# toandaominh1997/EfficientDet.Pytorch

Measured on NVIDIA H100. Metric: EfficientDet-D0 512x512 images/sec (fwd+bwd), higher is better.
Workload: dtype f32

## Files before the change

efficientdet.pytorch_b200/csrc/conv_planes.cu:

```cuda
#include "tc_ptx.cuh"

#include <stdlib.h>

namespace effdet {

constexpr int kPlMaxLevels = 8;
constexpr int kPlThreads = 288;
constexpr int kPlA = 128 * 128;
template <int BN>
struct PlCfg {
    static constexpr int kStages = BN == 128 ? 3 : 4;
    static constexpr int kB = BN * 128;
    static constexpr int kStage = 2 * kPlA + 2 * kB;
    static constexpr int kSmem = kStages * kStage + kRowsBytes + 1024 + 256 + BN * 4;
};

struct PlLevel {
    int B, H, W;
    WgGeom g;
    int tile_begin;
    int nboxes;
    float* y;
    long long y_bstride;
    __nv_bfloat16* y_planes;
    const __nv_bfloat16* mask_planes;
    const float* residual;
    long long r_bstride;
};
struct PlArgs {
    PlLevel lv[kPlMaxLevels];
    int nlevels, total_tiles, ntn;
    int Cin, Cout, ksize, act, kblocks, opitch;
    const float* bias;
    float* colsum;
};
struct PlMaps {
    CUtensorMap x[kPlMaxLevels];
};

template <int BN>
__global__ void __launch_bounds__(kPlThreads, 1)
conv_planes_kernel(const __grid_constant__ PlMaps maps, const __grid_constant__ CUtensorMap wmap, const __grid_constant__ PlArgs P) {
    constexpr int kPlBN = BN, kPlStages = PlCfg<BN>::kStages, kPlB = PlCfg<BN>::kB, kPlStage = PlCfg<BN>::kStage;
    extern __shared__ uint8_t smem_raw[];
    uint8_t* smem = smem_raw + ((1024u - (smem_u32(smem_raw) & 1023u)) & 1023u);
    float* rows_buf = reinterpret_cast<float*>(smem + kPlStages * kPlStage);
    uint64_t* full_bar = reinterpret_cast<uint64_t*>(smem + kPlStages * kPlStage + kRowsBytes);
    uint64_t* empty_bar = full_bar + kPlStages;
    float* chan = reinterpret_cast<float*>(smem + kPlStages * kPlStage + kRowsBytes + 256);

    const int warp = threadIdx.x >> 5, lane = threadIdx.x & 31;
    const int taps = P.ksize * P.ksize, pad = P.ksize / 2;
    const int KT = taps * P.kblocks;
    if (threadIdx.x == 0) {
        for (int s = 0; s < kPlStages; ++s) {
            mbar_init(&full_bar[s], 1);
            mbar_init(&empty_bar[s], 8);
        }
        fence_barrier_init();
        tma_prefetch_desc(&wmap);
    }
    __syncthreads();

    auto decode = [&](int unit, int& l, int& box0, int& n0) {
        const int mt = unit / P.ntn;
        n0 = (unit - mt * P.ntn) * kPlBN;
        l = 0;
        while (l + 1 < P.nlevels && mt >= P.lv[l + 1].tile_begin) ++l;
        box0 = (mt - P.lv[l].tile_begin) * (128 / P.lv[l].g.kstage);
    };

    if (warp == 8) {
        if (lane == 0) {
            uint32_t it = 0;
            for (int unit = blockIdx.x; unit < P.total_tiles; unit += gridDim.x) {
                int l, box0, n0;
                decode(unit, l, box0, n0);
                const PlLevel& L = P.lv[l];
                const int ks = L.g.kstage, nbox = 128 / ks;
                const int nvalid = min(nbox, L.nboxes - box0);
                for (int kt = 0; kt < KT; ++kt, ++it) {
                    const int s = it % kPlStages;
                    const uint32_t ph = (it / kPlStages) & 1;
                    const int tap = kt / P.kblocks, kb = kt - tap * P.kblocks;
                    const int dy = tap / P.ksize - pad, dx = tap % P.ksize - pad;
                    mbar_wait(&empty_bar[s], ph ^ 1);
                    uint8_t* a_hi = smem + s * kPlStage;
                    uint8_t* b_hi = a_hi + 2 * kPlA;
                    mbar_arrive_expect_tx(&full_bar[s], (uint32_t)(2 * nvalid * ks * 128 + 2 * kPlB));
                    for (int q = 0; q < nvalid; ++q) {
                        int ch = box0 + q;
                        const int bx = ch % L.g.nbx;
                        ch /= L.g.nbx;
                        const int by = ch % L.g.nby;
                        const int bb = ch / L.g.nby;
                        const int x0 = bx * L.g.Wb + dx, y0 = by * L.g.Hb + dy, b0 = bb * L.g.Bb;
                        tma_load_5d(a_hi + q * ks * 128, &maps.x[l], &full_bar[s], kb * 64, x0, y0, b0, 0);
                        tma_load_5d(a_hi + kPlA + q * ks * 128, &maps.x[l], &full_bar[s], kb * 64, x0, y0, b0, 1);
                    }
                    tma_load_3d(b_hi, &wmap, &full_bar[s], kt * 64, n0, 0);
                    tma_load_3d(b_hi + kPlB, &wmap, &full_bar[s], kt * 64, n0, 1);
                }
            }
        }
    } else {
        constexpr int NB = kPlBN / 64;
        const int g = warp >> 2;
        const int etid = threadIdx.x;
        const int quarter = 2 * g + (warp & 1), half = (warp >> 1) & 1;
        const int r = quarter * 32 + lane;
        uint32_t it = 0;
        int chan_n0 = -1;
        for (int unit = blockIdx.x; unit < P.total_tiles; unit += gridDim.x) {
            int l, box0, n0;
            decode(unit, l, box0, n0);
            const PlLevel& L = P.lv[l];
            float d[NB][32];
            for (int kt = 0; kt < KT; ++kt, ++it) {
                const int s = it % kPlStages;
                const uint32_t ph = (it / kPlStages) & 1;
                mbar_wait(&full_bar[s], ph);
                const uint32_t sa = smem_u32(smem + s * kPlStage) + g * 64 * 128;
                const uint32_t sb = smem_u32(smem + s * kPlStage) + 2 * kPlA;
                wgmma_fence();
#pragma unroll
                for (int k = 0; k < 4; ++k)
                    wg_mma3<NB, 0>(d, sa + k * 32, sa + kPlA + k * 32, sb + k * 32, sb + kPlB + k * 32, 16, 1024, (kt | k) != 0);
                wgmma_commit();
                wgmma_wait<1>();
                if (kt > 0 && lane == 0) mbar_arrive(&empty_bar[(it - 1) % kPlStages]);
            }
            wgmma_wait<0>();
            if (lane == 0) mbar_arrive(&empty_bar[(it - 1) % kPlStages]);
            if (n0 != chan_n0) {
                named_bar_sync(1, 256);
                for (int i = etid; i < kPlBN; i += 256) chan[i] = (n0 + i < P.Cout && P.bias) ? __ldg(P.bias + n0 + i) : 0.f;
                named_bar_sync(1, 256);
                chan_n0 = n0;
            }
            const int ks = L.g.kstage;
            const int q = r / ks, i = r - q * ks;
            int ch = box0 + q;
            bool row_ok = ch < L.nboxes;
            const int bx = ch % L.g.nbx;
            ch /= L.g.nbx;
            const int by = ch % L.g.nby;
            const int bb = ch / L.g.nby;
            const int wh = L.g.Wb * L.g.Hb;
            const int bi = i / wh, rem = i - bi * wh;
            const int yy = rem / L.g.Wb, xx = rem - yy * L.g.Wb;
            const int b = bb * L.g.Bb + bi, y = by * L.g.Hb + yy, x = bx * L.g.Wb + xx;
            row_ok = row_ok && b < L.B;
            const long long pixb = (long long)y * L.W + x;
            const long long pix = (long long)b * L.H * L.W + pixb;
            const long long plane = (long long)L.B * L.H * L.W * P.opitch;
            const int ncols = min(kPlBN, P.Cout - n0);
            const int nchunks = (ncols + 31) >> 5;
#pragma unroll
            for (int jb = 0; jb < NB; ++jb) {
                float v[32];
                wg_rows<2>(d[jb], rows_buf, g, v);
                const int cc = 2 * jb + half;
                if (cc >= nchunks) continue;
                const int nb = n0 + cc * 32;
#pragma unroll
                for (int k = 0; k < 32; ++k) {
                    float t = v[k] + chan[cc * 32 + k];
                    if (P.act == EFFDET_ACT_RELU) t = fmaxf(t, 0.f);
                    else if (P.act == EFFDET_ACT_SIGMOID) t = sigmoidf_(t);
                    v[k] = t;
                }
                if (row_ok && L.residual) {
#pragma unroll
                    for (int k4 = 0; k4 < 8; ++k4) {
                        if (nb + k4 * 4 >= P.Cout) break;
                        const float4 rv = ldg4(L.residual + (long long)b * L.r_bstride + pixb * P.Cout + nb + k4 * 4);
                        v[k4 * 4] += rv.x; v[k4 * 4 + 1] += rv.y; v[k4 * 4 + 2] += rv.z; v[k4 * 4 + 3] += rv.w;
                    }
                }
                if (row_ok && L.mask_planes) {
                    const __nv_bfloat16* mh = L.mask_planes + pix * P.opitch + nb;
#pragma unroll
                    for (int k8 = 0; k8 < 4; ++k8) {
                        if (nb + k8 * 8 >= P.Cout) break;
                        const uint4 hv = __ldg(reinterpret_cast<const uint4*>(mh + k8 * 8));
                        const uint4 lv = __ldg(reinterpret_cast<const uint4*>(mh + plane + k8 * 8));
                        const uint32_t hw[4] = {hv.x, hv.y, hv.z, hv.w}, lw[4] = {lv.x, lv.y, lv.z, lv.w};
#pragma unroll
                        for (int e = 0; e < 8; ++e) {
                            const uint32_t hb = (hw[e >> 1] >> ((e & 1) * 16)) & 0xffffu, lb = (lw[e >> 1] >> ((e & 1) * 16)) & 0xffffu;
                            const bool pos = (hb & 0x7fffu) ? !(hb & 0x8000u) : ((lb & 0x7fffu) && !(lb & 0x8000u));
                            if (!pos) v[k8 * 8 + e] = 0.f;
                        }
                    }
                }
                if (!row_ok) {
#pragma unroll
                    for (int k = 0; k < 32; ++k) v[k] = 0.f;
                }
                if (row_ok && L.y) {
                    float* yo = L.y + (long long)b * L.y_bstride + pixb * P.Cout + nb;
#pragma unroll
                    for (int k4 = 0; k4 < 8; ++k4) {
                        if (nb + k4 * 4 >= P.Cout) break;
                        st4(yo + k4 * 4, make_float4(v[k4 * 4], v[k4 * 4 + 1], v[k4 * 4 + 2], v[k4 * 4 + 3]));
                    }
                }
                if (row_ok && L.y_planes) {
                    __nv_bfloat16* ph = L.y_planes + pix * P.opitch + nb;
#pragma unroll
                    for (int k8 = 0; k8 < 4; ++k8) {
                        if (nb + k8 * 8 >= P.Cout) break;
                        uint4 hi, lo;
                        split8(make_float4(v[k8 * 8], v[k8 * 8 + 1], v[k8 * 8 + 2], v[k8 * 8 + 3]),
                               make_float4(v[k8 * 8 + 4], v[k8 * 8 + 5], v[k8 * 8 + 6], v[k8 * 8 + 7]), hi, lo);
                        *reinterpret_cast<uint4*>(ph + k8 * 8) = hi;
                        *reinterpret_cast<uint4*>(ph + plane + k8 * 8) = lo;
                    }
                }
                if (P.colsum) {
#pragma unroll
                    for (int off = 16; off >= 1; off >>= 1) {
                        const bool upper = (lane & off) != 0;
#pragma unroll
                        for (int k = 0; k < off; ++k) {
                            const float send = upper ? v[k] : v[k + off];
                            const float keep = upper ? v[k + off] : v[k];
                            v[k] = keep + __shfl_xor_sync(0xffffffffu, send, off);
                        }
                    }
                    if (nb + lane < P.Cout) atomicAdd(P.colsum + nb + lane, v[0]);
                }
            }
        }
    }
}

__global__ void __launch_bounds__(256) to_planes_kernel(const float* __restrict__ x, long long x_bstride, const float* __restrict__ prob,
                                                        long long p_bstride, __nv_bfloat16* __restrict__ out, float* __restrict__ colsum,
                                                        int B, int HW, int C, int pitch, int rows_per_block) {
    __shared__ float red[256 * 8];
    const int cv8 = pitch / 8;
    const int cvb = cv8 < 256 ? cv8 : 256;
    const int rows = 256 / cvb;
    const int tr = threadIdx.x / cvb, tc = threadIdx.x - tr * cvb;
    const int j = blockIdx.y * cvb + tc;
    const bool active = tr < rows && j < cv8;
    const long long nrows = (long long)B * HW;
    const long long plane = nrows * pitch;
    float s[8];
#pragma unroll
    for (int i = 0; i < 8; ++i) s[i] = 0.f;
    if (active) {
        const int c = j * 8;
        const long long r_begin = (long long)blockIdx.x * rows_per_block;
        const long long r_end = min(nrows, r_begin + rows_per_block);
        for (long long row = r_begin + tr; row < r_end; row += rows) {
            const int b = (int)(row / HW);
            const long long pix = row - (long long)b * HW;
            float4 v0 = f4zero(), v1 = f4zero();
            if (c < C) {
                const float* q = x + (long long)b * x_bstride + pix * C + c;
                v0 = ldg4(q);
                if (c + 4 < C) v1 = ldg4(q + 4);
                if (prob) {
                    const float* pp = prob + (long long)b * p_bstride + pix * C + c;
                    const float4 p0 = ldg4(pp);
                    v0 = make_float4(v0.x * p0.x * (1.f - p0.x), v0.y * p0.y * (1.f - p0.y), v0.z * p0.z * (1.f - p0.z),
                                     v0.w * p0.w * (1.f - p0.w));
                    if (c + 4 < C) {
                        const float4 p1 = ldg4(pp + 4);
                        v1 = make_float4(v1.x * p1.x * (1.f - p1.x), v1.y * p1.y * (1.f - p1.y), v1.z * p1.z * (1.f - p1.z),
                                         v1.w * p1.w * (1.f - p1.w));
                    }
                }
            }
            uint4 hi, lo;
            split8(v0, v1, hi, lo);
            *reinterpret_cast<uint4*>(out + row * pitch + c) = hi;
            *reinterpret_cast<uint4*>(out + plane + row * pitch + c) = lo;
            s[0] += v0.x; s[1] += v0.y; s[2] += v0.z; s[3] += v0.w;
            s[4] += v1.x; s[5] += v1.y; s[6] += v1.z; s[7] += v1.w;
        }
    }
    if (colsum == nullptr) return;
#pragma unroll
    for (int i = 0; i < 8; ++i) red[threadIdx.x * 8 + i] = s[i];
    __syncthreads();
    if (tr == 0 && j < cv8) {
#pragma unroll
        for (int i = 0; i < 8; ++i) {
            float acc = 0.f;
            for (int rr = 0; rr < rows; ++rr) acc += red[(rr * cvb + tc) * 8 + i];
            const int c = j * 8 + i;
            if (c < C) atomicAdd(colsum + c, acc);
        }
    }
}

}

using namespace effdet;

extern "C" int effdet_to_planes(const float* x, int64_t x_bstride, const float* prob, int64_t p_bstride, void* planes,
                                float* colsum, int B, int HW, int C, int device, effdet_stream_t stream) {
    EFFDET_REQUIRE(x && planes && B > 0 && HW > 0 && C > 0 && C % 4 == 0, "to_planes: bad arguments");
    EFFDET_REQUIRE(aligned16(x) && aligned16(prob) && aligned16(planes) && x_bstride % 4 == 0 && p_bstride % 4 == 0,
                   "to_planes: alignment");
    EFFDET_DEVICE(device);
    const int pitch = (C + 7) / 8 * 8;
    const int cv8 = pitch / 8;
    const int cvb = cv8 < 256 ? cv8 : 256;
    const int rows = 256 / cvb;
    const long long nrows = (long long)B * HW;
    long long rpb = (nrows + num_sms() * 4 - 1) / (num_sms() * 4);
    if (rpb < (long long)rows * 8) rpb = (long long)rows * 8;
    dim3 grid(cdiv(nrows, rpb), cdiv(cv8, cvb));
    to_planes_kernel<<<grid, 256, 0, (cudaStream_t)stream>>>(x, x_bstride, prob, p_bstride, (__nv_bfloat16*)planes, colsum, B, HW, C,
                                                            pitch, (int)rpb);
    return launch_status("to_planes_kernel");
}

extern "C" int effdet_conv_planes_multi(const effdet_conv_planes_args* levels, int nlevels, int device, effdet_stream_t stream) {
    EFFDET_REQUIRE(levels && nlevels >= 1 && nlevels <= kPlMaxLevels, "conv_planes_multi: 1..%d levels", kPlMaxLevels);
    const effdet_conv_planes_args* a0 = &levels[0];
    EFFDET_REQUIRE(a0->w_tc && (a0->ksize == 1 || a0->ksize == 3) && a0->Cin % 4 == 0 && a0->Cout % 4 == 0 && a0->Cin >= 8 &&
                       a0->Cout >= 8,
                   "conv_planes_multi: needs the bf16 weight pack, k in {1,3}, channels %% 4 == 0");
    EncodeTiledFn enc = encode_fn();
    if (!enc) return fail(EFFDET_ERR_UNSUPPORTED, "conv_planes_multi: cuTensorMapEncodeTiled unavailable");
    EFFDET_DEVICE(device);
    PlMaps maps;
    PlArgs P;
    memset(&P, 0, sizeof(P));
    const int opitch = (a0->Cout + 7) / 8 * 8, ipitch = (a0->Cin + 7) / 8 * 8;
    int tiles = 0;
    for (int l = 0; l < nlevels; ++l) {
        const effdet_conv_planes_args* a = &levels[l];
        EFFDET_REQUIRE(a->x_planes && (a->y || a->y_planes), "conv_planes_multi: null tensor");
        EFFDET_REQUIRE(a->Cin == a0->Cin && a->Cout == a0->Cout && a->ksize == a0->ksize && a->act == a0->act && a->w_tc == a0->w_tc &&
                           a->bias == a0->bias && a->colsum == a0->colsum,
                       "conv_planes_multi: all levels must share weights, bias, channels and activation");
        EFFDET_REQUIRE(aligned16(a->x_planes) && aligned16(a->y) && aligned16(a->y_planes) && aligned16(a->mask_planes) &&
                           aligned16(a->residual) && a->y_bstride % 4 == 0 && a->r_bstride % 4 == 0,
                       "conv_planes_multi: alignment");
        PlLevel& L = P.lv[l];
        L.B = a->B; L.H = a->H; L.W = a->W;
        if (!wg_geometry(a->B, a->H, a->W, &L.g))
            return fail(EFFDET_ERR_UNSUPPORTED, "conv_planes_multi: a %dx%dx%d map has no legal pixel box (check effdet_wgrad_tc_geometry_ok)",
                        a->B, a->H, a->W);
        L.nboxes = L.g.nbx * L.g.nby * L.g.nbb;
        L.tile_begin = tiles;
        tiles += cdiv(L.nboxes, 128 / L.g.kstage);
        L.y = a->y; L.y_bstride = a->y_bstride;
        L.y_planes = (__nv_bfloat16*)a->y_planes;
        L.mask_planes = (const __nv_bfloat16*)a->mask_planes;
        L.residual = a->residual; L.r_bstride = a->r_bstride;
        int s = planes_map(enc, &maps.x[l], const_cast<void*>(a->x_planes), a->B, a->H, a->W, a->Cin, ipitch, L.g);
        if (s) return s;
    }
    for (int l = nlevels; l < kPlMaxLevels; ++l) {
        maps.x[l] = maps.x[0];
        P.lv[l].tile_begin = tiles;
    }
    const int taps = a0->ksize * a0->ksize;
    const int kpad = conv_tc_kpad(a0->Cin);
    const int BN = a0->Cout <= 64 ? 64 : 128;
    CUtensorMap wmap;
    {
        const cuuint64_t gdim[3] = {(cuuint64_t)taps * kpad, (cuuint64_t)a0->Cout, 2};
        const cuuint64_t gstr[2] = {(cuuint64_t)taps * kpad * 2, (cuuint64_t)a0->Cout * taps * kpad * 2};
        const cuuint32_t box[3] = {64, (cuuint32_t)BN, 1};
        const cuuint32_t estr[3] = {1, 1, 1};
        CUresult r = enc(&wmap, CU_TENSOR_MAP_DATA_TYPE_BFLOAT16, 3, const_cast<void*>(a0->w_tc), gdim, gstr, box, estr,
                         CU_TENSOR_MAP_INTERLEAVE_NONE, CU_TENSOR_MAP_SWIZZLE_128B, CU_TENSOR_MAP_L2_PROMOTION_L2_256B,
                         CU_TENSOR_MAP_FLOAT_OOB_FILL_NONE);
        if (r != CUDA_SUCCESS) return fail(EFFDET_ERR_LAUNCH, "conv_planes_multi: tensor map of the weights failed (%d)", (int)r);
    }
    P.nlevels = nlevels;
    P.ntn = cdiv(a0->Cout, BN);
    P.total_tiles = tiles * P.ntn;
    P.Cin = a0->Cin; P.Cout = a0->Cout; P.ksize = a0->ksize; P.act = a0->act;
    P.kblocks = kpad / 64;
    P.opitch = opitch;
    P.bias = a0->bias;
    P.colsum = a0->colsum;
    const int grid = P.total_tiles < num_sms() ? P.total_tiles : num_sms();
#define EFFDET_PL_LAUNCH(BN_)                                                                                              \
    do {                                                                                                                  \
        cudaError_t e = cudaFuncSetAttribute(conv_planes_kernel<BN_>, cudaFuncAttributeMaxDynamicSharedMemorySize,         \
                                             PlCfg<BN_>::kSmem);                                                          \
        if (e != cudaSuccess) return fail(EFFDET_ERR_LAUNCH, "conv_planes_multi: smem opt-in: %s", cudaGetErrorString(e)); \
        conv_planes_kernel<BN_><<<grid, kPlThreads, PlCfg<BN_>::kSmem, (cudaStream_t)stream>>>(maps, wmap, P);             \
    } while (0)
    if (BN == 64) EFFDET_PL_LAUNCH(64);
    else EFFDET_PL_LAUNCH(128);
#undef EFFDET_PL_LAUNCH
    return launch_status("conv_planes_kernel");
}
```

efficientdet.pytorch_b200/csrc/conv_tc.cu:

```cuda
#include "tc_ptx.cuh"

#include <stdlib.h>

namespace effdet {

constexpr int kTcThreads = 288;
constexpr int kTcProducers = 256;
constexpr int kFwdThreads = 288;
constexpr int kFwdProducers = 256;
constexpr int kTileM = 128;
constexpr int kTileK = 64;

template <int BN, int STAGES>
struct FwdSmem {
    static constexpr int kA = kTileM * 128;
    static constexpr int kB = BN * 128;
    static constexpr int kStage = 2 * kA + 2 * kB;
    static constexpr int kChan = 3 * BN * 4;
    static constexpr int kBytes = STAGES * kStage + 1024  + 256  + kChan;
};

template <int BN, int STAGES, bool MB>
__device__ __forceinline__ void conv_tc_body(const CUtensorMap& wmap, const effdet_conv_args& p, const int M, const int HW,
                                             const int kblocks, const int m0, const int n0) {
// ... 670 lines not shown
#define EFFDET_TC_LAUNCH(BN_, ST_)                                                                                         \
    do {                                                                                                                  \
        if (mb) EFFDET_TC_LAUNCH1(BN_, ST_, true);                                                                        \
        else EFFDET_TC_LAUNCH1(BN_, ST_, false);                                                                          \
    } while (0)
    if (KT <= 2) {
        if (BN == 64) EFFDET_TC_LAUNCH(64, 1);
        else EFFDET_TC_LAUNCH(128, 1);
    } else {
        if (BN == 64) EFFDET_TC_LAUNCH(64, 4);
        else EFFDET_TC_LAUNCH(128, 3);
    }
#undef EFFDET_TC_LAUNCH
#undef EFFDET_TC_LAUNCH1
    return launch_status("conv_tc_kernel");
}


int conv_tc_multi_launch(const effdet_conv_args* levels, int nlevels, cudaStream_t st) {
    EncodeTiledFn enc = encode_fn();
    if (!enc) return fail(EFFDET_ERR_UNSUPPORTED, "conv2d_multi(tc): cuTensorMapEncodeTiled unavailable");
    const effdet_conv_args* a = &levels[0];
    const int taps = a->ksize * a->ksize;
    const int kpad = conv_tc_kpad(a->Cin);
    const int kblocks = kpad / kTileK;
    const int BN = a->Cout <= 64 ? 64 : 128;
    CUtensorMap map;
    const cuuint64_t gdim[3] = {(cuuint64_t)taps * kpad, (cuuint64_t)a->Cout, 2};
    const cuuint64_t gstr[2] = {(cuuint64_t)taps * kpad * 2, (cuuint64_t)a->Cout * taps * kpad * 2};
    const cuuint32_t box[3] = {(cuuint32_t)kTileK, (cuuint32_t)BN, 1};
    const cuuint32_t estr[3] = {1, 1, 1};
    CUresult r = enc(&map, CU_TENSOR_MAP_DATA_TYPE_BFLOAT16, 3, const_cast<void*>(a->w_tc), gdim, gstr, box, estr,
                     CU_TENSOR_MAP_INTERLEAVE_NONE, CU_TENSOR_MAP_SWIZZLE_128B, CU_TENSOR_MAP_L2_PROMOTION_L2_256B,
                     CU_TENSOR_MAP_FLOAT_OOB_FILL_NONE);
    if (r != CUDA_SUCCESS) return fail(EFFDET_ERR_LAUNCH, "conv2d_multi(tc): cuTensorMapEncodeTiled failed (%d)", (int)r);
    ConvMultiArgs ma;
    memset(&ma, 0, sizeof(ma));
    ma.nlevels = nlevels;
    int tiles = 0;
    for (int l = 0; l < nlevels; ++l) {
        ma.lv[l] = levels[l];
        ma.tile_begin[l] = tiles;
        tiles += cdiv((long long)levels[l].B * levels[l].H * levels[l].W, kTileM);
    }
    for (int l = nlevels; l <= kMaxLevels; ++l) ma.tile_begin[l] = tiles;
    dim3 grid(tiles, cdiv(a->Cout, BN));
#define EFFDET_TCM_LAUNCH(BN_, ST_)                                                                                        \
    do {                                                                                                                  \
        cudaError_t e = cudaFuncSetAttribute(conv_tc_multi_kernel<BN_, ST_>, cudaFuncAttributeMaxDynamicSharedMemorySize,  \
                                             FwdSmem<BN_, ST_>::kBytes);                                                  \
        if (e != cudaSuccess) return fail(EFFDET_ERR_LAUNCH, "conv2d_multi(tc): smem opt-in: %s", cudaGetErrorString(e)); \
        conv_tc_multi_kernel<BN_, ST_><<<grid, kFwdThreads, FwdSmem<BN_, ST_>::kBytes, st>>>(map, ma, kblocks);            \
    } while (0)
    if (BN == 64) EFFDET_TCM_LAUNCH(64, 4);
    else EFFDET_TCM_LAUNCH(128, 3);
#undef EFFDET_TCM_LAUNCH
    return launch_status("conv_tc_multi_kernel");
}

bool wgrad_tc_eligible(const effdet_wgrad_args* a) {
    if (a->precision != 1 || a->Cin % 4 || a->Cout % 4 || a->Cin < 16 || a->Cout < 16) return false;
    WgGeom g;
    const bool tma_ok = (a->ws_x || a->x_planes) && (a->ws_dy || a->dy_planes) && wg_geometry(a->B, a->H, a->W, &g);
    return tma_ok || (!a->a_scale && !a->in_scale && !a->dy_planes && !a->x_planes);
}

bool wg_geometry(int B, int H, int W, WgGeom* g) {
    const int Wb = W <= 64 ? W : 64;
    if (W % Wb) return false;
    int Hb = 1;
    for (int h = 1; h <= H && Wb * h <= 64; ++h)
        if (H % h == 0) Hb = h;
    int Bb = 64 / (Wb * Hb);
    if (Bb < 1) Bb = 1;
    if (Bb > B) Bb = B;
    const int ks = Wb * Hb * Bb;
    if (ks < 16 || ks % 16) return false;
    g->Wb = Wb; g->Hb = Hb; g->Bb = Bb;
    g->nbx = W / Wb; g->nby = H / Hb; g->nbb = (B + Bb - 1) / Bb;
    g->kstage = ks;
    return true;
}

int planes_map(EncodeTiledFn enc, CUtensorMap* map, void* base, int B, int H, int W, int C, int pitch, const WgGeom& g) {
    const cuuint64_t gdim[5] = {(cuuint64_t)C, (cuuint64_t)W, (cuuint64_t)H, (cuuint64_t)B, 2};
    const cuuint64_t gstr[4] = {(cuuint64_t)pitch * 2, (cuuint64_t)W * pitch * 2, (cuuint64_t)H * W * pitch * 2,
                                (cuuint64_t)B * H * W * pitch * 2};
    const cuuint32_t box[5] = {64, (cuuint32_t)g.Wb, (cuuint32_t)g.Hb, (cuuint32_t)g.Bb, 1};
    const cuuint32_t estr[5] = {1, 1, 1, 1, 1};
    CUresult r = enc(map, CU_TENSOR_MAP_DATA_TYPE_BFLOAT16, 5, base, gdim, gstr, box, estr, CU_TENSOR_MAP_INTERLEAVE_NONE,
                     CU_TENSOR_MAP_SWIZZLE_128B, CU_TENSOR_MAP_L2_PROMOTION_L2_256B, CU_TENSOR_MAP_FLOAT_OOB_FILL_NONE);
    if (r != CUDA_SUCCESS) return fail(EFFDET_ERR_LAUNCH, "wgrad(tc): cuTensorMapEncodeTiled failed (%d)", (int)r);
    return EFFDET_OK;
}

static int wgrad_tc2_launch(const effdet_wgrad_args* a, cudaStream_t st) {
    WgGeom g;
    EncodeTiledFn enc = encode_fn();
    if (!enc || !(a->ws_x || a->x_planes) || !(a->ws_dy || a->dy_planes) || !wg_geometry(a->B, a->H, a->W, &g)) return 1;
    const int HW = a->H * a->W;
    const int cin_pad = conv_tc_kpad(a->Cin), cout_pad = conv_tc_kpad(a->Cout);
    int s = EFFDET_OK;
    if (!a->x_planes) {
        int blocks = cdiv((long long)a->B * HW * (cin_pad / 8), 256);
        if (blocks > num_sms() * 16) blocks = num_sms() * 16;
        split_planes_kernel<<<blocks, 256, 0, st>>>(a->x, a->x_bstride, a->a_scale, (__nv_bfloat16*)a->ws_x, a->B, HW, a->Cin, cin_pad,
                                                    a->in_scale, a->in_shift);
        s = launch_status("split_planes_kernel");
        if (s) return s;
    }
    CUtensorMap mdy, mx;
    if (a->dy_planes) {
        if ((s = planes_map(enc, &mdy, const_cast<void*>(a->dy_planes), a->B, a->H, a->W, a->Cout, (a->Cout + 7) / 8 * 8, g))) return s;
    } else {
        if ((s = split_dy_launch(a, cout_pad, st))) return s;
        if ((s = planes_map(enc, &mdy, a->ws_dy, a->B, a->H, a->W, cout_pad, cout_pad, g))) return s;
    }
    if (a->x_planes) {
        if ((s = planes_map(enc, &mx, const_cast<void*>(a->x_planes), a->B, a->H, a->W, a->Cin, (a->Cin + 7) / 8 * 8, g))) return s;
    } else {
        if ((s = planes_map(enc, &mx, a->ws_x, a->B, a->H, a->W, cin_pad, cin_pad, g))) return s;
    }
    const int taps = a->ksize * a->ksize;
    const int BC = a->Cin > 64 ? 256 : 64;
    const int ctiles = cdiv(a->Cin, BC), ntiles = cdiv(a->Cout, kTileM);
    const int nchunks = g.nbx * g.nby * g.nbb;
    int splits = (num_sms() * 2) / (ctiles * ntiles * taps);
    if (splits < 1) splits = 1;
    if (splits > cdiv(nchunks, 4)) splits = cdiv(nchunks, 4);
    int cps = cdiv(nchunks, splits);
    splits = cdiv(nchunks, cps);
    dim3 grid(ctiles * ntiles, taps, splits);
    cudaError_t e;
    if (BC == 256) {
        constexpr int ST = 2;
        e = cudaFuncSetAttribute(wgrad_tc2_kernel<256, ST>, cudaFuncAttributeMaxDynamicSharedMemorySize, WgSmem<256, ST>::kBytes);
        if (e != cudaSuccess) return fail(EFFDET_ERR_LAUNCH, "wgrad(tc): smem opt-in: %s", cudaGetErrorString(e));
        wgrad_tc2_kernel<256, ST><<<grid, kTcThreads, WgSmem<256, ST>::kBytes, st>>>(mdy, mx, *a, g, cps, ctiles);
    } else {
        constexpr int ST = 4;
        e = cudaFuncSetAttribute(wgrad_tc2_kernel<64, ST>, cudaFuncAttributeMaxDynamicSharedMemorySize, WgSmem<64, ST>::kBytes);
        if (e != cudaSuccess) return fail(EFFDET_ERR_LAUNCH, "wgrad(tc): smem opt-in: %s", cudaGetErrorString(e));
        wgrad_tc2_kernel<64, ST><<<grid, kTcThreads, WgSmem<64, ST>::kBytes, st>>>(mdy, mx, *a, g, cps, ctiles);
    }
    return launch_status("wgrad_tc2_kernel");
}

int wgrad_tc2_multi_launch(const effdet_wgrad_args* levels, int nlevels, cudaStream_t st) {
    EncodeTiledFn enc = encode_fn();
    if (!enc || nlevels > kWgMaxLevels) return 1;
    WgMaps maps;
    WgMultiArgs ma;
    memset(&ma, 0, sizeof(ma));
    const effdet_wgrad_args* a0 = &levels[0];
    const int cin_pad = conv_tc_kpad(a0->Cin), cout_pad = conv_tc_kpad(a0->Cout);
    int chunks = 0;
    for (int l = 0; l < nlevels; ++l) {
        const effdet_wgrad_args* a = &levels[l];
        if (!(a->ws_x || a->x_planes) || !(a->ws_dy || a->dy_planes) || a->a_scale || a->in_scale ||
            !wg_geometry(a->B, a->H, a->W, &ma.g[l]))
            return 1;
        ma.chunk_begin[l] = chunks;
        chunks += ma.g[l].nbx * ma.g[l].nby * ma.g[l].nbb;
    }
    for (int l = nlevels; l <= kWgMaxLevels; ++l) ma.chunk_begin[l] = chunks;
    ma.nlevels = nlevels;
    ma.dw = a0->dw;
    ma.Cin = a0->Cin; ma.Cout = a0->Cout; ma.ksize = a0->ksize;
    for (int l = 0; l < nlevels; ++l) {
        const effdet_wgrad_args* a = &levels[l];
        const int HW = a->H * a->W;
        int s = EFFDET_OK;
        if (a->x_planes) {
            if ((s = planes_map(enc, &maps.x[l], const_cast<void*>(a->x_planes), a->B, a->H, a->W, a->Cin, (a->Cin + 7) / 8 * 8, ma.g[l])))
// ... 168 lines not shown
```

efficientdet.pytorch_b200/csrc/tc_ptx.cuh:

```cuda
#pragma once
#include "common.cuh"

#include <cuda.h>
#include <cuda_bf16.h>
#include <type_traits>

namespace effdet {

__device__ __forceinline__ uint32_t smem_u32(const void* p) { return (uint32_t)__cvta_generic_to_shared(p); }

__device__ __forceinline__ void mbar_init(uint64_t* bar, uint32_t count) {
    asm volatile("mbarrier.init.shared::cta.b64 [%0], %1;" ::"r"(smem_u32(bar)), "r"(count));
}
__device__ __forceinline__ void mbar_arrive(uint64_t* bar) {
    asm volatile("mbarrier.arrive.shared::cta.b64 _, [%0];" ::"r"(smem_u32(bar)) : "memory");
}
__device__ __forceinline__ void mbar_arrive_expect_tx(uint64_t* bar, uint32_t bytes) {
    asm volatile("mbarrier.arrive.expect_tx.shared::cta.b64 _, [%0], %1;" ::"r"(smem_u32(bar)), "r"(bytes) : "memory");
}
__device__ __forceinline__ void mbar_wait(uint64_t* bar, uint32_t parity) {
    const uint32_t a = smem_u32(bar);
    uint32_t done;
    do {
        asm volatile(
            "{\n\t.reg .pred p;\n\t"
            "mbarrier.try_wait.parity.shared::cta.b64 p, [%1], %2;\n\t"
            "selp.u32 %0, 1, 0, p;\n\t}"
            : "=r"(done)
            : "r"(a), "r"(parity)
            : "memory");
    } while (!done);
}
__device__ __forceinline__ void fence_barrier_init() { asm volatile("fence.mbarrier_init.release.cluster;" ::: "memory"); }
__device__ __forceinline__ void fence_proxy_async() { asm volatile("fence.proxy.async.shared::cta;" ::: "memory"); }
__device__ __forceinline__ void tma_load_3d(void* dst, const CUtensorMap* map, uint64_t* bar, int c0, int c1, int c2) {
    asm volatile(
        "cp.async.bulk.tensor.3d.shared::cluster.global.tile.mbarrier::complete_tx::bytes [%0], [%1, {%3, %4, %5}], [%2];"
        ::"r"(smem_u32(dst)), "l"(reinterpret_cast<uint64_t>(map)), "r"(smem_u32(bar)), "r"(c0), "r"(c1), "r"(c2)
        : "memory");
}

__device__ __forceinline__ void tma_load_5d(void* dst, const CUtensorMap* map, uint64_t* bar, int c0, int c1, int c2, int c3, int c4) {
    asm volatile(
        "cp.async.bulk.tensor.5d.shared::cluster.global.tile.mbarrier::complete_tx::bytes [%0], [%1, {%3, %4, %5, %6, %7}], [%2];"
        ::"r"(smem_u32(dst)), "l"(reinterpret_cast<uint64_t>(map)), "r"(smem_u32(bar)), "r"(c0), "r"(c1), "r"(c2), "r"(c3), "r"(c4)
        : "memory");
}


__device__ __forceinline__ uint64_t gmma_desc(uint32_t smem_addr, uint32_t lbo_bytes, uint32_t sbo_bytes) {
    return (uint64_t)((smem_addr >> 4) & 0x3FFF) | ((uint64_t)((lbo_bytes >> 4) & 0x3FFF) << 16) |
           ((uint64_t)((sbo_bytes >> 4) & 0x3FFF) << 32) | (1ull << 62);
}
__device__ __forceinline__ void wgmma_fence() { asm volatile("wgmma.fence.sync.aligned;" ::: "memory"); }
__device__ __forceinline__ void wgmma_commit() { asm volatile("wgmma.commit_group.sync.aligned;" ::: "memory"); }
template <int N>
__device__ __forceinline__ void wgmma_wait() {
    asm volatile("wgmma.wait_group.sync.aligned %0;" ::"n"(N) : "memory");
}
#define EFFDET_WG_D8(a, o) "+f"(a[o]), "+f"(a[o + 1]), "+f"(a[o + 2]), "+f"(a[o + 3]), "+f"(a[o + 4]), "+f"(a[o + 5]), \
                           "+f"(a[o + 6]), "+f"(a[o + 7])
#define EFFDET_WG_D32(a) EFFDET_WG_D8(a, 0), EFFDET_WG_D8(a, 8), EFFDET_WG_D8(a, 16), EFFDET_WG_D8(a, 24)
template <int MN>
__device__ __forceinline__ void wgmma_bf16(float (&d)[1][32], uint64_t desc_a, uint64_t desc_b, uint32_t accumulate) {
    asm volatile(
        "{\n\t.reg .pred p;\n\t"
        "setp.ne.b32 p, %34, 0;\n\t"
        "wgmma.mma_async.sync.aligned.m64n64k16.f32.bf16.bf16 {"
        "%0, %1, %2, %3, %4, %5, %6, %7, %8, %9, %10, %11, %12, %13, %14, %15, "
        "%16, %17, %18, %19, %20, %21, %22, %23, %24, %25, %26, %27, %28, %29, %30, %31"
        "}, %32, %33, p, 1, 1, %35, %35;\n\t}"
        : EFFDET_WG_D32(d[0])
        : "l"(desc_a), "l"(desc_b), "r"(accumulate), "n"(MN)
        : "memory");
}
template <int MN>
__device__ __forceinline__ void wgmma_bf16(float (&d)[2][32], uint64_t desc_a, uint64_t desc_b, uint32_t accumulate) {
    asm volatile(
        "{\n\t.reg .pred p;\n\t"
        "setp.ne.b32 p, %66, 0;\n\t"
        "wgmma.mma_async.sync.aligned.m64n128k16.f32.bf16.bf16 {"
        "%0, %1, %2, %3, %4, %5, %6, %7, %8, %9, %10, %11, %12, %13, %14, %15, "
        "%16, %17, %18, %19, %20, %21, %22, %23, %24, %25, %26, %27, %28, %29, %30, %31, "
        "%32, %33, %34, %35, %36, %37, %38, %39, %40, %41, %42, %43, %44, %45, %46, %47, "
        "%48, %49, %50, %51, %52, %53, %54, %55, %56, %57, %58, %59, %60, %61, %62, %63"
        "}, %64, %65, p, 1, 1, %67, %67;\n\t}"
        : EFFDET_WG_D32(d[0]), EFFDET_WG_D32(d[1])
        : "l"(desc_a), "l"(desc_b), "r"(accumulate), "n"(MN)
        : "memory");
}
template <int MN>
__device__ __forceinline__ void wgmma_bf16(float (&d)[4][32], uint64_t desc_a, uint64_t desc_b, uint32_t accumulate) {
    asm volatile(
        "{\n\t.reg .pred p;\n\t"
        "setp.ne.b32 p, %130, 0;\n\t"
        "wgmma.mma_async.sync.aligned.m64n256k16.f32.bf16.bf16 {"
        "%0, %1, %2, %3, %4, %5, %6, %7, %8, %9, %10, %11, %12, %13, %14, %15, "
        "%16, %17, %18, %19, %20, %21, %22, %23, %24, %25, %26, %27, %28, %29, %30, %31, "
        "%32, %33, %34, %35, %36, %37, %38, %39, %40, %41, %42, %43, %44, %45, %46, %47, "
        "%48, %49, %50, %51, %52, %53, %54, %55, %56, %57, %58, %59, %60, %61, %62, %63, "
        "%64, %65, %66, %67, %68, %69, %70, %71, %72, %73, %74, %75, %76, %77, %78, %79, "
        "%80, %81, %82, %83, %84, %85, %86, %87, %88, %89, %90, %91, %92, %93, %94, %95, "
        "%96, %97, %98, %99, %100, %101, %102, %103, %104, %105, %106, %107, %108, %109, %110, %111, "
        "%112, %113, %114, %115, %116, %117, %118, %119, %120, %121, %122, %123, %124, %125, %126, %127"
        "}, %128, %129, p, 1, 1, %131, %131;\n\t}"
        : EFFDET_WG_D32(d[0]), EFFDET_WG_D32(d[1]), EFFDET_WG_D32(d[2]), EFFDET_WG_D32(d[3])
        : "l"(desc_a), "l"(desc_b), "r"(accumulate), "n"(MN)
        : "memory");
}
#undef EFFDET_WG_D32
#undef EFFDET_WG_D8
template <int NB, int MN>
__device__ __forceinline__ void wg_mma3(float (&d)[NB][32], uint32_t a_hi, uint32_t a_lo, uint32_t b_hi, uint32_t b_lo,
                                        uint32_t lbo, uint32_t sbo, uint32_t accumulate) {
    const uint64_t dah = gmma_desc(a_hi, lbo, sbo), dal = gmma_desc(a_lo, lbo, sbo);
    const uint64_t dbh = gmma_desc(b_hi, lbo, sbo), dbl = gmma_desc(b_lo, lbo, sbo);
    wgmma_bf16<MN>(d, dal, dbh, accumulate);
    wgmma_bf16<MN>(d, dah, dbl, 1);
    wgmma_bf16<MN>(d, dah, dbh, 1);
}
template <int KS, int NB>
__device__ __forceinline__ void wg_mma3_mn_steps(float (&d)[NB][32], uint32_t a_hi, uint32_t a_lo, uint32_t b_hi, uint32_t b_lo,
                                                 uint32_t group, uint32_t accumulate) {
    wgmma_fence();
#pragma unroll
    for (int k = 0; k < KS; ++k) {
        const uint32_t ko = k * 2 * 1024;
        wg_mma3<NB, 1>(d, a_hi + ko, a_lo + ko, b_hi + ko, b_lo + ko, group, 1024, accumulate | k);
    }
}
template <int... KS, class F>
__device__ __forceinline__ void with_count(const int n, F&& f) {
    (void)((n == KS && (f(std::integral_constant<int, KS>()), true)) || ...);
}

__device__ __forceinline__ void named_bar_sync(int id, int nthreads) {
    asm volatile("bar.sync %0, %1;" ::"r"(id), "r"(nthreads) : "memory");
}

constexpr int kRowsPitch = 68;
constexpr int kRowsBytes = 64 * kRowsPitch * 4;
template <int NWG>
__device__ __forceinline__ void wg_rows(const float (&d)[32], float* buf, const int g, float (&out)[32]) {
    const int w = (threadIdx.x >> 5) & 3, lane = threadIdx.x & 31;
#pragma unroll 1
    for (int turn = 0; turn < NWG; ++turn) {
        named_bar_sync(1, NWG * 128);
        if (turn != g) continue;
#pragma unroll
        for (int i = 0; i < 32; i += 2) {
            const int row = 16 * w + (lane >> 2) + 8 * ((i >> 1) & 1), col = 8 * (i >> 2) + 2 * (lane & 3);
            *reinterpret_cast<float2*>(buf + row * kRowsPitch + col) = make_float2(d[i], d[i + 1]);
        }
        named_bar_sync(2 + g, 128);
        const float* src = buf + ((w & 1) * 32 + lane) * kRowsPitch + (w >> 1) * 32;
#pragma unroll
        for (int q = 0; q < 8; ++q) {
            const float4 v = *reinterpret_cast<const float4*>(src + 4 * q);
            out[4 * q] = v.x; out[4 * q + 1] = v.y; out[4 * q + 2] = v.z; out[4 * q + 3] = v.w;
        }
    }
}

__device__ __forceinline__ void split8(const float4 a, const float4 b, uint4& hi, uint4& lo) {
    const float f[8] = {a.x, a.y, a.z, a.w, b.x, b.y, b.z, b.w};
    uint32_t h[4], l[4];
#pragma unroll
    for (int i = 0; i < 4; ++i) {
        const __nv_bfloat162 hh = __floats2bfloat162_rn(f[2 * i], f[2 * i + 1]);
        const float r0 = f[2 * i] - __low2float(hh), r1 = f[2 * i + 1] - __high2float(hh);
        const __nv_bfloat162 ll = __floats2bfloat162_rn(r0, r1);
        h[i] = *reinterpret_cast<const uint32_t*>(&hh);
        l[i] = *reinterpret_cast<const uint32_t*>(&ll);
    }
    hi = make_uint4(h[0], h[1], h[2], h[3]);
    lo = make_uint4(l[0], l[1], l[2], l[3]);
}


__device__ __forceinline__ void tma_load_2d(void* dst, const CUtensorMap* map, uint64_t* bar, int c0, int c1) {
    asm volatile(
        "cp.async.bulk.tensor.2d.shared::cluster.global.tile.mbarrier::complete_tx::bytes [%0], [%1, {%3, %4}], [%2];"
        ::"r"(smem_u32(dst)), "l"(reinterpret_cast<uint64_t>(map)), "r"(smem_u32(bar)), "r"(c0), "r"(c1)
        : "memory");
}
__device__ __forceinline__ void tma_store_2d(const CUtensorMap* map, const void* src, int c0, int c1) {
    asm volatile("cp.async.bulk.tensor.2d.global.shared::cta.tile.bulk_group [%0, {%2, %3}], [%1];"
                 ::"l"(reinterpret_cast<uint64_t>(map)), "r"(smem_u32(src)), "r"(c0), "r"(c1)
                 : "memory");
}
__device__ __forceinline__ void tma_store_commit() { asm volatile("cp.async.bulk.commit_group;" ::: "memory"); }
template <int N>
__device__ __forceinline__ void tma_store_wait_read() {
    asm volatile("cp.async.bulk.wait_group.read %0;" ::"n"(N) : "memory");
}
__device__ __forceinline__ void tma_prefetch_desc(const CUtensorMap* map) {
    asm volatile("prefetch.tensormap [%0];" ::"l"(reinterpret_cast<uint64_t>(map)) : "memory");
}
typedef CUresult (*EncodeTiledFn)(CUtensorMap*, CUtensorMapDataType, cuuint32_t, void*, const cuuint64_t*, const cuuint64_t*,
                                  const cuuint32_t*, const cuuint32_t*, CUtensorMapInterleave, CUtensorMapSwizzle,
                                  CUtensorMapL2promotion, CUtensorMapFloatOOBfill);
EncodeTiledFn encode_fn();
int conv_tc_kpad(int k);

struct WgGeom {
    int Wb, Hb, Bb;
    int nbx, nby, nbb;
    int kstage;
};
bool wg_geometry(int B, int H, int W, WgGeom* g);
int planes_map(EncodeTiledFn enc, CUtensorMap* map, void* base, int B, int H, int W, int C, int pitch, const WgGeom& g);

}
```

Measured before the change: 506.7.

## Add BN=256 conv-planes variant with K=32 stages and split wide/narrow launches

Adds a 256-wide output-channel tile configuration for the planes conv kernel. To fit shared memory it halves the K chunk to 32 (64-byte swizzle), uses 384 threads, and rebalances registers with setmaxnreg between the producer and consumer warps. The host now splits the tile range into a wide launch sized to whole waves of SMs and a remainder launch with the old 64/128 configs. The aim is more reuse of A tiles per weight load for wide Cout layers, at the cost of twice as many K iterations and barriers, a second kernel launch, and register pressure.

```diff
diff --git a/efficientdet.pytorch_b200/csrc/conv_planes.cu b/efficientdet.pytorch_b200/csrc/conv_planes.cu
--- a/efficientdet.pytorch_b200/csrc/conv_planes.cu
+++ b/efficientdet.pytorch_b200/csrc/conv_planes.cu
@@ -5,13 +5,15 @@
 namespace effdet {
 
 constexpr int kPlMaxLevels = 8;
-constexpr int kPlThreads = 288;
-constexpr int kPlA = 128 * 128;
 template <int BN>
 struct PlCfg {
+    static constexpr int kK = BN == 256 ? 32 : 64;
+    static constexpr int kRow = kK * 2;
     static constexpr int kStages = BN == 128 ? 3 : 4;
-    static constexpr int kB = BN * 128;
-    static constexpr int kStage = 2 * kPlA + 2 * kB;
+    static constexpr int kThreads = BN == 256 ? 384 : 288;
+    static constexpr int kA = 128 * kRow;
+    static constexpr int kB = BN * kRow;
+    static constexpr int kStage = 2 * kA + 2 * kB;
     static constexpr int kSmem = kStages * kStage + kRowsBytes + 1024 + 256 + BN * 4;
 };
 
@@ -30,6 +32,7 @@
 struct PlArgs {
     PlLevel lv[kPlMaxLevels];
     int nlevels, total_tiles, ntn;
+    int tile0;
     int Cin, Cout, ksize, act, kblocks, opitch;
     const float* bias;
     float* colsum;
@@ -39,9 +42,10 @@
 };
 
 template <int BN>
-__global__ void __launch_bounds__(kPlThreads, 1)
+__global__ void __launch_bounds__(PlCfg<BN>::kThreads, 1)
 conv_planes_kernel(const __grid_constant__ PlMaps maps, const __grid_constant__ CUtensorMap wmap, const __grid_constant__ PlArgs P) {
-    constexpr int kPlBN = BN, kPlStages = PlCfg<BN>::kStages, kPlB = PlCfg<BN>::kB, kPlStage = PlCfg<BN>::kStage;
+    constexpr int kPlBN = BN, kPlStages = PlCfg<BN>::kStages, kPlA = PlCfg<BN>::kA, kPlB = PlCfg<BN>::kB, kPlStage = PlCfg<BN>::kStage;
+    constexpr int kK = PlCfg<BN>::kK, kRow = PlCfg<BN>::kRow;
     extern __shared__ uint8_t smem_raw[];
     uint8_t* smem = smem_raw + ((1024u - (smem_u32(smem_raw) & 1023u)) & 1023u);
     float* rows_buf = reinterpret_cast<float*>(smem + kPlStages * kPlStage);
@@ -63,15 +67,16 @@
     __syncthreads();
 
     auto decode = [&](int unit, int& l, int& box0, int& n0) {
-        const int mt = unit / P.ntn;
-        n0 = (unit - mt * P.ntn) * kPlBN;
+        const int mt = P.tile0 + unit / P.ntn;
+        n0 = (unit % P.ntn) * kPlBN;
         l = 0;
         while (l + 1 < P.nlevels && mt >= P.lv[l + 1].tile_begin) ++l;
         box0 = (mt - P.lv[l].tile_begin) * (128 / P.lv[l].g.kstage);
     };
 
-    if (warp == 8) {
-        if (lane == 0) {
+    if (warp >= 8) {
+        if constexpr (PlCfg<BN>::kThreads == 384) setmaxnreg_dec<40>();
+        if (warp == 8 && lane == 0) {
             uint32_t it = 0;
             for (int unit = blockIdx.x; unit < P.total_tiles; unit += gridDim.x) {
                 int l, box0, n0;
@@ -87,7 +92,7 @@
                     mbar_wait(&empty_bar[s], ph ^ 1);
                     uint8_t* a_hi = smem + s * kPlStage;
                     uint8_t* b_hi = a_hi + 2 * kPlA;
-                    mbar_arrive_expect_tx(&full_bar[s], (uint32_t)(2 * nvalid * ks * 128 + 2 * kPlB));
+                    mbar_arrive_expect_tx(&full_bar[s], (uint32_t)(2 * nvalid * ks * kRow + 2 * kPlB));
                     for (int q = 0; q < nvalid; ++q) {
                         int ch = box0 + q;
                         const int bx = ch % L.g.nbx;
@@ -95,15 +100,16 @@
                         const int by = ch % L.g.nby;
                         const int bb = ch / L.g.nby;
                         const int x0 = bx * L.g.Wb + dx, y0 = by * L.g.Hb + dy, b0 = bb * L.g.Bb;
-                        tma_load_5d(a_hi + q * ks * 128, &maps.x[l], &full_bar[s], kb * 64, x0, y0, b0, 0);
-                        tma_load_5d(a_hi + kPlA + q * ks * 128, &maps.x[l], &full_bar[s], kb * 64, x0, y0, b0, 1);
-                    }
-                    tma_load_3d(b_hi, &wmap, &full_bar[s], kt * 64, n0, 0);
-                    tma_load_3d(b_hi + kPlB, &wmap, &full_bar[s], kt * 64, n0, 1);
+                        tma_load_5d(a_hi + q * ks * kRow, &maps.x[l], &full_bar[s], kb * kK, x0, y0, b0, 0);
+                        tma_load_5d(a_hi + kPlA + q * ks * kRow, &maps.x[l], &full_bar[s], kb * kK, x0, y0, b0, 1);
+                    }
+                    tma_load_3d(b_hi, &wmap, &full_bar[s], kt * kK, n0, 0);
+                    tma_load_3d(b_hi + kPlB, &wmap, &full_bar[s], kt * kK, n0, 1);
                 }
             }
         }
     } else {
+        if constexpr (PlCfg<BN>::kThreads == 384) setmaxnreg_inc<232>();
         constexpr int NB = kPlBN / 64;
         const int g = warp >> 2;
         const int etid = threadIdx.x;
@@ -120,12 +126,13 @@
                 const int s = it % kPlStages;
                 const uint32_t ph = (it / kPlStages) & 1;
                 mbar_wait(&full_bar[s], ph);
-                const uint32_t sa = smem_u32(smem + s * kPlStage) + g * 64 * 128;
+                const uint32_t sa = smem_u32(smem + s * kPlStage) + g * 64 * kRow;
                 const uint32_t sb = smem_u32(smem + s * kPlStage) + 2 * kPlA;
                 wgmma_fence();
 #pragma unroll
-                for (int k = 0; k < 4; ++k)
-                    wg_mma3<NB, 0>(d, sa + k * 32, sa + kPlA + k * 32, sb + k * 32, sb + kPlB + k * 32, 16, 1024, (kt | k) != 0);
+                for (int k = 0; k < kK / 16; ++k)
+                    wg_mma3<NB, 0, kRow>(d, sa + k * 32, sa + kPlA + k * 32, sb + k * 32, sb + kPlB + k * 32, 16, 8 * kRow,
+                                         (kt | k) != 0);
                 wgmma_commit();
                 wgmma_wait<1>();
                 if (kt > 0 && lane == 0) mbar_arrive(&empty_bar[(it - 1) % kPlStages]);
@@ -156,10 +163,13 @@
             const long long plane = (long long)L.B * L.H * L.W * P.opitch;
             const int ncols = min(kPlBN, P.Cout - n0);
             const int nchunks = (ncols + 31) >> 5;
-#pragma unroll
+            constexpr int kUnroll = NB == 4 ? 1 : NB;
+#pragma unroll (kUnroll)
             for (int jb = 0; jb < NB; ++jb) {
                 float v[32];
-                wg_rows<2>(d[jb], rows_buf, g, v);
+#pragma unroll
+                for (int j = 0; j < NB; ++j)
+                    if (j == jb) wg_rows<2>(d[j], rows_buf, g, v);
                 const int cc = 2 * jb + half;
                 if (cc >= nchunks) continue;
                 const int nb = n0 + cc * 32;
@@ -321,6 +331,39 @@
     return launch_status("to_planes_kernel");
 }
 
+template <int BN>
+static int pl_launch(const effdet_conv_planes_args* levels, EncodeTiledFn enc, int taps, int kpad, PlArgs P, int tile0, int ntiles,
+                     cudaStream_t stream) {
+    constexpr int kK = PlCfg<BN>::kK;
+    const effdet_conv_planes_args* a0 = &levels[0];
+    PlMaps maps;
+    for (int l = 0; l < P.nlevels; ++l) {
+        const effdet_conv_planes_args* a = &levels[l];
+        int s = planes_map(enc, &maps.x[l], const_cast<void*>(a->x_planes), a->B, a->H, a->W, a->Cin, (a->Cin + 7) / 8 * 8,
+                           P.lv[l].g, kK);
+        if (s) return s;
+    }
+    for (int l = P.nlevels; l < kPlMaxLevels; ++l) maps.x[l] = maps.x[0];
+    CUtensorMap wmap;
+    const cuuint64_t gdim[3] = {(cuuint64_t)taps * kpad, (cuuint64_t)a0->Cout, 2};
+    const cuuint64_t gstr[2] = {(cuuint64_t)taps * kpad * 2, (cuuint64_t)a0->Cout * taps * kpad * 2};
+    const cuuint32_t box[3] = {(cuuint32_t)kK, (cuuint32_t)BN, 1};
+    const cuuint32_t estr[3] = {1, 1, 1};
+    CUresult r = enc(&wmap, CU_TENSOR_MAP_DATA_TYPE_BFLOAT16, 3, const_cast<void*>(a0->w_tc), gdim, gstr, box, estr,
+                     CU_TENSOR_MAP_INTERLEAVE_NONE, kK == 64 ? CU_TENSOR_MAP_SWIZZLE_128B : CU_TENSOR_MAP_SWIZZLE_64B,
+                     CU_TENSOR_MAP_L2_PROMOTION_L2_256B, CU_TENSOR_MAP_FLOAT_OOB_FILL_NONE);
+    if (r != CUDA_SUCCESS) return fail(EFFDET_ERR_LAUNCH, "conv_planes_multi: tensor map of the weights failed (%d)", (int)r);
+    P.kblocks = kpad / kK;
+    P.ntn = cdiv(a0->Cout, BN);
+    P.tile0 = tile0;
+    P.total_tiles = ntiles * P.ntn;
+    const int grid = P.total_tiles < num_sms() ? P.total_tiles : num_sms();
+    cudaError_t e = cudaFuncSetAttribute(conv_planes_kernel<BN>, cudaFuncAttributeMaxDynamicSharedMemorySize, PlCfg<BN>::kSmem);
+    if (e != cudaSuccess) return fail(EFFDET_ERR_LAUNCH, "conv_planes_multi: smem opt-in: %s", cudaGetErrorString(e));
+    conv_planes_kernel<BN><<<grid, PlCfg<BN>::kThreads, PlCfg<BN>::kSmem, stream>>>(maps, wmap, P);
+    return launch_status("conv_planes_kernel");
+}
+
 extern "C" int effdet_conv_planes_multi(const effdet_conv_planes_args* levels, int nlevels, int device, effdet_stream_t stream) {
     EFFDET_REQUIRE(levels && nlevels >= 1 && nlevels <= kPlMaxLevels, "conv_planes_multi: 1..%d levels", kPlMaxLevels);
     const effdet_conv_planes_args* a0 = &levels[0];
@@ -330,10 +373,9 @@
     EncodeTiledFn enc = encode_fn();
     if (!enc) return fail(EFFDET_ERR_UNSUPPORTED, "conv_planes_multi: cuTensorMapEncodeTiled unavailable");
     EFFDET_DEVICE(device);
-    PlMaps maps;
     PlArgs P;
     memset(&P, 0, sizeof(P));
-    const int opitch = (a0->Cout + 7) / 8 * 8, ipitch = (a0->Cin + 7) / 8 * 8;
+    const int opitch = (a0->Cout + 7) / 8 * 8;
     int tiles = 0;
     for (int l = 0; l < nlevels; ++l) {
         const effdet_conv_planes_args* a = &levels[l];
@@ -356,45 +398,26 @@
         L.y_planes = (__nv_bfloat16*)a->y_planes;
         L.mask_planes = (const __nv_bfloat16*)a->mask_planes;
         L.residual = a->residual; L.r_bstride = a->r_bstride;
-        int s = planes_map(enc, &maps.x[l], const_cast<void*>(a->x_planes), a->B, a->H, a->W, a->Cin, ipitch, L.g);
-        if (s) return s;
-    }
-    for (int l = nlevels; l < kPlMaxLevels; ++l) {
-        maps.x[l] = maps.x[0];
-        P.lv[l].tile_begin = tiles;
-    }
+    }
+    for (int l = nlevels; l < kPlMaxLevels; ++l) P.lv[l].tile_begin = tiles;
     const int taps = a0->ksize * a0->ksize;
     const int kpad = conv_tc_kpad(a0->Cin);
-    const int BN = a0->Cout <= 64 ? 64 : 128;
-    CUtensorMap wmap;
-    {
-        const cuuint64_t gdim[3] = {(cuuint64_t)taps * kpad, (cuuint64_t)a0->Cout, 2};
-        const cuuint64_t gstr[2] = {(cuuint64_t)taps * kpad * 2, (cuuint64_t)a0->Cout * taps * kpad * 2};
-        const cuuint32_t box[3] = {64, (cuuint32_t)BN, 1};
-        const cuuint32_t estr[3] = {1, 1, 1};
-        CUresult r = enc(&wmap, CU_TENSOR_MAP_DATA_TYPE_BFLOAT16, 3, const_cast<void*>(a0->w_tc), gdim, gstr, box, estr,
-                         CU_TENSOR_MAP_INTERLEAVE_NONE, CU_TENSOR_MAP_SWIZZLE_128B, CU_TENSOR_MAP_L2_PROMOTION_L2_256B,
-                         CU_TENSOR_MAP_FLOAT_OOB_FILL_NONE);
-        if (r != CUDA_SUCCESS) return fail(EFFDET_ERR_LAUNCH, "conv_planes_multi: tensor map of the weights failed (%d)", (int)r);
-    }
     P.nlevels = nlevels;
-    P.ntn = cdiv(a0->Cout, BN);
-    P.total_tiles = tiles * P.ntn;
     P.Cin = a0->Cin; P.Cout = a0->Cout; P.ksize = a0->ksize; P.act = a0->act;
-    P.kblocks = kpad / 64;
     P.opitch = opitch;
     P.bias = a0->bias;
     P.colsum = a0->colsum;
-    const int grid = P.total_tiles < num_sms() ? P.total_tiles : num_sms();
-#define EFFDET_PL_LAUNCH(BN_)                                                                                              \
-    do {                                                                                                                  \
-        cudaError_t e = cudaFuncSetAttribute(conv_planes_kernel<BN_>, cudaFuncAttributeMaxDynamicSharedMemorySize,         \
-                                             PlCfg<BN_>::kSmem);                                                          \
-        if (e != cudaSuccess) return fail(EFFDET_ERR_LAUNCH, "conv_planes_multi: smem opt-in: %s", cudaGetErrorString(e)); \
-        conv_planes_kernel<BN_><<<grid, kPlThreads, PlCfg<BN_>::kSmem, (cudaStream_t)stream>>>(maps, wmap, P);             \
-    } while (0)
-    if (BN == 64) EFFDET_PL_LAUNCH(64);
-    else EFFDET_PL_LAUNCH(128);
-#undef EFFDET_PL_LAUNCH
-    return launch_status("conv_planes_kernel");
-}
+    const int Cout = a0->Cout;
+    int wide_tiles = 0;
+    if (Cout > 128 && cdiv(Cout, 256) * 256 == cdiv(Cout, 128) * 128) {
+        const long long units = (long long)tiles * cdiv(Cout, 256);
+        if (units > num_sms()) wide_tiles = (int)(units / num_sms() * num_sms() / cdiv(Cout, 256));
+    }
+    int s = 0;
+    if (wide_tiles > 0) s = pl_launch<256>(levels, enc, taps, kpad, P, 0, wide_tiles, (cudaStream_t)stream);
+    if (s == 0 && wide_tiles < tiles) {
+        if (Cout <= 64) s = pl_launch<64>(levels, enc, taps, kpad, P, wide_tiles, tiles - wide_tiles, (cudaStream_t)stream);
+        else s = pl_launch<128>(levels, enc, taps, kpad, P, wide_tiles, tiles - wide_tiles, (cudaStream_t)stream);
+    }
+    return s;
+}
diff --git a/efficientdet.pytorch_b200/csrc/conv_tc.cu b/efficientdet.pytorch_b200/csrc/conv_tc.cu
--- a/efficientdet.pytorch_b200/csrc/conv_tc.cu
+++ b/efficientdet.pytorch_b200/csrc/conv_tc.cu
@@ -776,14 +776,15 @@
     return true;
 }
 
-int planes_map(EncodeTiledFn enc, CUtensorMap* map, void* base, int B, int H, int W, int C, int pitch, const WgGeom& g) {
+int planes_map(EncodeTiledFn enc, CUtensorMap* map, void* base, int B, int H, int W, int C, int pitch, const WgGeom& g, int kc) {
     const cuuint64_t gdim[5] = {(cuuint64_t)C, (cuuint64_t)W, (cuuint64_t)H, (cuuint64_t)B, 2};
     const cuuint64_t gstr[4] = {(cuuint64_t)pitch * 2, (cuuint64_t)W * pitch * 2, (cuuint64_t)H * W * pitch * 2,
                                 (cuuint64_t)B * H * W * pitch * 2};
-    const cuuint32_t box[5] = {64, (cuuint32_t)g.Wb, (cuuint32_t)g.Hb, (cuuint32_t)g.Bb, 1};
+    const cuuint32_t box[5] = {(cuuint32_t)kc, (cuuint32_t)g.Wb, (cuuint32_t)g.Hb, (cuuint32_t)g.Bb, 1};
     const cuuint32_t estr[5] = {1, 1, 1, 1, 1};
     CUresult r = enc(map, CU_TENSOR_MAP_DATA_TYPE_BFLOAT16, 5, base, gdim, gstr, box, estr, CU_TENSOR_MAP_INTERLEAVE_NONE,
-                     CU_TENSOR_MAP_SWIZZLE_128B, CU_TENSOR_MAP_L2_PROMOTION_L2_256B, CU_TENSOR_MAP_FLOAT_OOB_FILL_NONE);
+                     kc == 64 ? CU_TENSOR_MAP_SWIZZLE_128B : CU_TENSOR_MAP_SWIZZLE_64B, CU_TENSOR_MAP_L2_PROMOTION_L2_256B,
+                     CU_TENSOR_MAP_FLOAT_OOB_FILL_NONE);
     if (r != CUDA_SUCCESS) return fail(EFFDET_ERR_LAUNCH, "wgrad(tc): cuTensorMapEncodeTiled failed (%d)", (int)r);
     return EFFDET_OK;
 }
diff --git a/efficientdet.pytorch_b200/csrc/tc_ptx.cuh b/efficientdet.pytorch_b200/csrc/tc_ptx.cuh
--- a/efficientdet.pytorch_b200/csrc/tc_ptx.cuh
+++ b/efficientdet.pytorch_b200/csrc/tc_ptx.cuh
@@ -48,9 +48,11 @@
 }
 
 
+template <int SW = 128>
 __device__ __forceinline__ uint64_t gmma_desc(uint32_t smem_addr, uint32_t lbo_bytes, uint32_t sbo_bytes) {
+    static_assert(SW == 128 || SW == 64, "swizzle: 128 or 64 bytes");
     return (uint64_t)((smem_addr >> 4) & 0x3FFF) | ((uint64_t)((lbo_bytes >> 4) & 0x3FFF) << 16) |
-           ((uint64_t)((sbo_bytes >> 4) & 0x3FFF) << 32) | (1ull << 62);
+           ((uint64_t)((sbo_bytes >> 4) & 0x3FFF) << 32) | ((SW == 128 ? 1ull : 2ull) << 62);
 }
 __device__ __forceinline__ void wgmma_fence() { asm volatile("wgmma.fence.sync.aligned;" ::: "memory"); }
 __device__ __forceinline__ void wgmma_commit() { asm volatile("wgmma.commit_group.sync.aligned;" ::: "memory"); }
@@ -110,11 +112,11 @@
 }
 #undef EFFDET_WG_D32
 #undef EFFDET_WG_D8
-template <int NB, int MN>
+template <int NB, int MN, int SW = 128>
 __device__ __forceinline__ void wg_mma3(float (&d)[NB][32], uint32_t a_hi, uint32_t a_lo, uint32_t b_hi, uint32_t b_lo,
                                         uint32_t lbo, uint32_t sbo, uint32_t accumulate) {
-    const uint64_t dah = gmma_desc(a_hi, lbo, sbo), dal = gmma_desc(a_lo, lbo, sbo);
-    const uint64_t dbh = gmma_desc(b_hi, lbo, sbo), dbl = gmma_desc(b_lo, lbo, sbo);
+    const uint64_t dah = gmma_desc<SW>(a_hi, lbo, sbo), dal = gmma_desc<SW>(a_lo, lbo, sbo);
+    const uint64_t dbh = gmma_desc<SW>(b_hi, lbo, sbo), dbl = gmma_desc<SW>(b_lo, lbo, sbo);
     wgmma_bf16<MN>(d, dal, dbh, accumulate);
     wgmma_bf16<MN>(d, dah, dbl, 1);
     wgmma_bf16<MN>(d, dah, dbh, 1);
@@ -132,6 +134,15 @@
 template <int... KS, class F>
 __device__ __forceinline__ void with_count(const int n, F&& f) {
     (void)((n == KS && (f(std::integral_constant<int, KS>()), true)) || ...);
+}
+
+template <int N>
+__device__ __forceinline__ void setmaxnreg_dec() {
+    asm volatile("setmaxnreg.dec.sync.aligned.u32 %0;" ::"n"(N));
+}
+template <int N>
+__device__ __forceinline__ void setmaxnreg_inc() {
+    asm volatile("setmaxnreg.inc.sync.aligned.u32 %0;" ::"n"(N));
 }
 
 __device__ __forceinline__ void named_bar_sync(int id, int nthreads) {
@@ -209,6 +220,7 @@
     int kstage;
 };
 bool wg_geometry(int B, int H, int W, WgGeom* g);
-int planes_map(EncodeTiledFn enc, CUtensorMap* map, void* base, int B, int H, int W, int C, int pitch, const WgGeom& g);
-
-}
+int planes_map(EncodeTiledFn enc, CUtensorMap* map, void* base, int B, int H, int W, int C, int pitch, const WgGeom& g,
+               int kc = 64);
+
+}
```

New measurement: 510.8, median of 6. No clear change (+0.8%).
